# tnibler/local-features

Hardware: AMD Instinct MI355X
Metric: MKD descriptors/sec (32x32 patch, 128-D) (higher is better)
Workload: dtype f32 (f16x3 split MFMA pooling)

## Files before the change

local-features_amd/csrc/mkd_ablate.h:

```cpp
#pragma once
#include <hip/hip_runtime.h>

namespace lfmkd {
namespace ablate {

#ifdef LF_ABLATE_BLOAD
constexpr bool kNoFragmentReads = true;
#else
constexpr bool kNoFragmentReads = false;
#endif
#ifdef LF_ABLATE_SPLIT
constexpr bool kNoSplit = true;
#else
constexpr bool kNoSplit = false;
#endif
#ifdef LF_ABLATE_MMA
constexpr bool kNoMma = true;
#else
constexpr bool kNoMma = false;
#endif
#ifdef LF_ABLATE_FRONT
constexpr bool kNoFrontEnd = true;
#else
constexpr bool kNoFrontEnd = false;
#endif
#ifdef LF_ABLATE_MUL_FIRST_TAP
constexpr bool kMulFirstTap = true;
#else
constexpr bool kMulFirstTap = false;
#endif
#ifdef LF_ABLATE_SYNC
constexpr bool kNoRowSync = true;
#else
constexpr bool kNoRowSync = false;
#endif
#ifdef LF_ABLATE_EPILOGUE
constexpr bool kNoEpilogue = true;
#else
constexpr bool kNoEpilogue = false;
#endif
#ifdef LF_ABLATE_FORCE_W4
constexpr bool kForceFourWaves = true;
#else
constexpr bool kForceFourWaves = false;
#endif
#ifdef LF_KP_ABLATE_PRODUCER
constexpr bool kNoProducer = true;
#else
constexpr bool kNoProducer = false;
#endif
#ifdef LF_KP_ABLATE_TAPS
constexpr bool kNoTaps = true;
#else
constexpr bool kNoTaps = false;
#endif
#ifdef LF_KP_PRODUCER_PRIO
constexpr int kProducerPrio = LF_KP_PRODUCER_PRIO;
#else
constexpr int kProducerPrio = 2;
#endif
#ifdef LF_KP_CONSUMER_PRIO
constexpr int kConsumerPrio = LF_KP_CONSUMER_PRIO;
#else
constexpr int kConsumerPrio = -1;
#endif

#ifdef LF_ABLATE_ROWS
constexpr int kRows = LF_ABLATE_ROWS;
#else
constexpr int kRows = 32;
#endif

#ifdef LF_PHASE_TIMING
constexpr bool kPhaseTiming = true;
#else
constexpr bool kPhaseTiming = false;
#endif
struct PhaseClock {
    unsigned long long clk[8] = {0, 0, 0, 0, 0, 0, 0, 0}, prev = 0;
    __device__ __forceinline__ void start() {
        if constexpr (kPhaseTiming) prev = __builtin_readcyclecounter();
    }
    __device__ __forceinline__ void mark(int i) {
        if constexpr (kPhaseTiming) {
            __builtin_amdgcn_sched_barrier(0);
            const unsigned long long t = __builtin_readcyclecounter();
            clk[i] += t - prev;
            prev = t;
            __builtin_amdgcn_sched_barrier(0);
        }
    }
    __device__ __forceinline__ void dump(float *out, int wave, int lane) const {
        if constexpr (kPhaseTiming) {
            __syncthreads();
            if (blockIdx.x == 0 && lane == 0)
                for (int i = 0; i < 8; ++i) out[wave * 128 + i] = (float)clk[i];
        }
    }
};

}
}
```

local-features_amd/csrc/mkd_describe.hip:

```cpp
#include <hip/hip_runtime.h>
#include <stdint.h>

#include <type_traits>

#include "mkd_ablate.h"
#include "mkd_device.h"
#include "mkd_sample.h"

namespace lfmkd {


namespace {

typedef _Float16 f16x8 __attribute__((ext_vector_type(8)));
typedef unsigned int u32x4 __attribute__((ext_vector_type(4)));
typedef float f32x2 __attribute__((ext_vector_type(2)));
__device__ __forceinline__ f32x2 pk_fma(f32x2 a, f32x2 b, f32x2 c) { return __builtin_elementwise_fma(a, b, c); }
__device__ __forceinline__ f32x2 pk_set(float v) { return f32x2{v, v}; }

__device__ __host__ constexpr bool f16_family(int pool) { return pool == LF_POOL_F16X3 || pool == LF_POOL_F16_FP6; }

__device__ __host__ constexpr bool fold_form(int pool) { return pool != LF_POOL_F16_FP6; }
constexpr int kTiles = 21;
constexpr int kAccTiles = 21, kUnfAccTiles = 24;
__device__ __host__ constexpr int acc_tiles(bool fold) { return fold ? kAccTiles : kUnfAccTiles; }
__device__ __host__ constexpr int lut_pieces(bool fold) { return fold ? 24 : 30; }
__device__ __host__ constexpr bool valu_odd_cart(int pool) { return pool == LF_POOL_F16X3; }
constexpr int kOddCartSums = 7;
constexpr int kPolarSlots = 10;

constexpr float kB0 = 0.0096f, kB1 = 0.2054f, kB2 = 0.5699f;

__device__ __host__ constexpr int row_bytes(bool fold) { return lut_pieces(fold) * 1024; }
__device__ __host__ constexpr int ring_off(bool fold) { return 2 * row_bytes(fold); }
constexpr int kRowBytes = row_bytes(true), kRingOff = ring_off(true);
constexpr int kRingSlots = 6;
[[maybe_unused]] constexpr int kSrcPatches = 0, kSrcKeypoints = 1, kSrcKeypointsSplit = 2;
constexpr int kRingSlotsKp = 12;
constexpr int kLevelTableBytes = 5 * kMaxPyrLevels * 4;

__device__ __forceinline__ float lane_fetch(int byte_addr, float v) {
    return __int_as_float(__builtin_amdgcn_ds_bpermute(byte_addr, __float_as_int(v)));
}

__device__ __forceinline__ void lds_dma16(const void *gsrc, void *ldst) {
    __builtin_amdgcn_global_load_lds((const __attribute__((address_space(1))) void *)gsrc,
                                     (__attribute__((address_space(3))) void *)ldst, 16, 0, 0);
}
__device__ __forceinline__ void lds_dma16_sv(const unsigned char *uniform_base, unsigned lane_off, void *ldst) {
    asm("" : "+s"(uniform_base));
    asm volatile("" : "+v"(lane_off));
    lds_dma16(uniform_base + lane_off, ldst);
}

template <int W, bool FOLD, bool ODDV>
__device__ __forceinline__ void issue_lut_row(const unsigned char *__restrict__ lut_rows, int row,
                                              unsigned char *lds_row, int wave, int lane) {
    static_assert(!ODDV || FOLD, "the folded forms' tiles");
    constexpr int kPieces = ODDV ? lut_pieces(FOLD) - 8 : lut_pieces(FOLD);
    const unsigned lane16 = (unsigned)lane * 16u;
#pragma unroll
    for (int j = 0; j < (kPieces + W - 1) / W; ++j) {
        if (kPieces % W == 0 || wave + W * j < kPieces) {
            const int i = wave + W * j, piece = ODDV ? i + 2 * (i >> 2) : i;
            const unsigned char *g = lut_rows + ((size_t)row * row_bytes(FOLD) + (size_t)piece * 1024);
            lds_dma16_sv(g, lane16, lds_row + piece * 1024);
        }
    }
}

constexpr int kWStepBytes = 16384;
__device__ __forceinline__ constexpr int wstage_slot(int step) { return step % 3 == 0 ? 0 : (step % 3 == 1 ? 32768 : 16384); }
static_assert(wstage_slot(0) + kWStepBytes <= row_bytes(true) && wstage_slot(10) >= row_bytes(false) &&
              wstage_slot(10) + kWStepBytes <= 2 * row_bytes(true), "both forms' row buffers");

template <int W>
__device__ __forceinline__ void issue_w_step(const unsigned char *__restrict__ wfrag, int step, unsigned char *lds,
                                             int wave, int lane) {
    const unsigned lane16 = (unsigned)lane * 16u;
    unsigned char *d = lds + wstage_slot(step);
#pragma unroll
    for (int j = 0; j < 16 / W; ++j) {
        const unsigned char *g = wfrag + ((size_t)step * kWStepBytes + (size_t)(wave + W * j) * 1024);
        lds_dma16_sv(g, lane16, d + (wave + W * j) * 1024);
    }
}

template <int N> __device__ __forceinline__ void wait_vmcnt() { asm volatile("s_waitcnt vmcnt(%0)" ::"n"(N) : "memory"); }

struct RawSrc { const unsigned char *base; unsigned lane_off; };
__device__ __forceinline__ constexpr int clamp_row(int row) { return row < 0 ? 0 : (row > 31 ? 31 : row); }
__device__ __forceinline__ void issue_raw_row(const RawSrc &src, int row, unsigned char *ring, int slot) {
    const unsigned char *g = src.base + row * 128;
    lds_dma16_sv(g, src.lane_off, ring + slot * 2048);
    lds_dma16_sv(g + 64, src.lane_off, ring + slot * 2048 + 1024);
}

#pragma clang fp contract(off)

__device__ __forceinline__ float max3_tiny(float a, float b) {
    return __builtin_fmaxf(__builtin_fmaxf(a, b), 1e-30f);
}

template <int ANGLE>
__device__ __forceinline__ void gradient_direction(f32x2 gx, f32x2 gy, f32x2 r2, f32x2 &ct, f32x2 &st) {
    if (ANGLE == LF_ANGLE_EXACT || ANGLE == LF_ANGLE_EXACT_ZERO) {
        const f32x2 inv = {__builtin_amdgcn_rsqf(r2.x), __builtin_amdgcn_rsqf(r2.y)};
        const f32x2 c = gx * inv, s = -gy * inv;
        const bool z0 = ANGLE == LF_ANGLE_EXACT ? r2.x == 0.f : gx.x == 0.f;
        const bool z1 = ANGLE == LF_ANGLE_EXACT ? r2.y == 0.f : gx.y == 0.f;
        ct = f32x2{z0 ? 1.f : c.x, z1 ? 1.f : c.y};
        st = f32x2{z0 ? 0.f : s.x, z1 ? 0.f : s.y};
    } else {
        const float ax0 = fabsf(gx.x), ay0 = fabsf(gy.x), ax1 = fabsf(gx.y), ay1 = fabsf(gy.y);
        const bool sw0 = ax0 < ay0 && gx.x != 0.f, sw1 = ax1 < ay1 && gx.y != 0.f;
        const f32x2 mn = {__builtin_fminf(ax0, ay0), __builtin_fminf(ax1, ay1)};
        const f32x2 mx = {max3_tiny(ax0, ay0), max3_tiny(ax1, ay1)};
        const f32x2 a = mn * f32x2{__builtin_amdgcn_rcpf(mx.x), __builtin_amdgcn_rcpf(mx.y)};
        const f32x2 s = a * a;
        f32x2 p = pk_fma(s, pk_set(-0.0117212f), pk_set(0.05265332f));
        p = pk_fma(s, p, pk_set(-0.11643287f));
        p = pk_fma(s, p, pk_set(0.19354346f));
        p = pk_fma(s, p, pk_set(-0.33262347f));
        p = pk_fma(s, p, pk_set(0.99997726f));
        p = a * p;
        const f32x2 p2 = p * p;
        f32x2 sn = pk_fma(p2, pk_set(-0.000195038549f), pk_set(0.0083320355f));
        sn = pk_fma(p2, sn, pk_set(-0.166666508f));
        sn = pk_fma(p2, sn, pk_set(1.f));
        sn = p * sn;
        f32x2 cs = pk_fma(p2, pk_set(-0.00135857589f), pk_set(0.0416550152f));
        cs = pk_fma(p2, cs, pk_set(-0.499998569f));
        cs = pk_fma(p2, cs, pk_set(1.f));
        const unsigned sgn = 0x80000000u;
        float cr0 = __uint_as_float(__float_as_uint(sw0 ? sn.x : cs.x) | (__float_as_uint(gx.x) & sgn));
        float cr1 = __uint_as_float(__float_as_uint(sw1 ? sn.y : cs.y) | (__float_as_uint(gx.y) & sgn));
        float sr0 = __uint_as_float(__float_as_uint(sw0 ? cs.x : sn.x) | (~__float_as_uint(gy.x) & sgn));
        float sr1 = __uint_as_float(__float_as_uint(sw1 ? cs.y : sn.y) | (~__float_as_uint(gy.y) & sgn));
        ct = f32x2{cr0, cr1};
        st = f32x2{sr0, sr1};
    }
}

template <int ANGLE>
__device__ __forceinline__ void gradient_direction4(const f32x2 (&gx)[4], const f32x2 (&gy)[4], const f32x2 (&r2)[4],
                                                    f32x2 (&ct)[4], f32x2 (&st)[4]) {
    if (ANGLE != LF_ANGLE_SHADER) {
#pragma unroll
        for (int e = 0; e < 4; ++e) gradient_direction<ANGLE>(gx[e], gy[e], r2[e], ct[e], st[e]);
        return;
    }
    f32x2 a[4], s[4], p[4], p2[4], sn[4], cs[4];
    bool sw0[4], sw1[4];
#pragma unroll
    for (int e = 0; e < 4; ++e) {
        const float ax0 = fabsf(gx[e].x), ay0 = fabsf(gy[e].x), ax1 = fabsf(gx[e].y), ay1 = fabsf(gy[e].y);
        sw0[e] = ax0 < ay0 && gx[e].x != 0.f;
        sw1[e] = ax1 < ay1 && gx[e].y != 0.f;
        const f32x2 mn = {__builtin_fminf(ax0, ay0), __builtin_fminf(ax1, ay1)};
        const f32x2 mx = {max3_tiny(ax0, ay0), max3_tiny(ax1, ay1)};
        a[e] = mn * f32x2{__builtin_amdgcn_rcpf(mx.x), __builtin_amdgcn_rcpf(mx.y)};
    }
#pragma unroll
    for (int e = 0; e < 4; ++e) s[e] = a[e] * a[e];
#pragma unroll
    for (int e = 0; e < 4; ++e) p[e] = pk_fma(s[e], pk_set(-0.0117212f), pk_set(0.05265332f));
#pragma unroll
    for (int e = 0; e < 4; ++e) p[e] = pk_fma(s[e], p[e], pk_set(-0.11643287f));
#pragma unroll
    for (int e = 0; e < 4; ++e) p[e] = pk_fma(s[e], p[e], pk_set(0.19354346f));
#pragma unroll
    for (int e = 0; e < 4; ++e) p[e] = pk_fma(s[e], p[e], pk_set(-0.33262347f));
#pragma unroll
    for (int e = 0; e < 4; ++e) p[e] = pk_fma(s[e], p[e], pk_set(0.99997726f));
#pragma unroll
    for (int e = 0; e < 4; ++e) p[e] = a[e] * p[e];
#pragma unroll
    for (int e = 0; e < 4; ++e) p2[e] = p[e] * p[e];
// ... 200 lines not shown
    float ext[12];
    const float l0 = lane_fetch(addr_l, vb[6]), l1 = lane_fetch(addr_l, vb[7]);
    const float r0 = lane_fetch(addr_r, vb[0]), r1 = lane_fetch(addr_r, vb[1]);
    ext[0] = has_l ? l0 : vb[0];
    ext[1] = has_l ? l1 : vb[0];
    ext[10] = has_r ? r0 : vb[7];
    ext[11] = has_r ? r1 : vb[7];
#pragma unroll
    for (int x = 0; x < 8; ++x) ext[2 + x] = vb[x];
#pragma unroll
    for (int x = 0; x < 8; ++x) {
        float s = ablate::kMulFirstTap ? kB0 * ext[x] : fmaf(kB0, ext[x], 0.0f);
        s = fmaf(kB1, ext[x + 1], s);
        s = fmaf(kB2, ext[x + 2], s);
        s = fmaf(kB1, ext[x + 3], s);
        s = fmaf(kB0, ext[x + 4], s);
        out[x] = s;
    }
    const float hl = lane_fetch(addr_l, out[7]), hr = lane_fetch(addr_r, out[0]);
    out_l = has_l ? hl : out[0];
    out_r = has_r ? hr : out[7];
}

template <class SlotOfTap>
__device__ __forceinline__ void blur_row_impl(const unsigned char *ring_lane, SlotOfTap slot_of_tap, int addr_l, int addr_r,
                                              bool has_l, bool has_r, float (&out)[8], float &out_l, float &out_r) {
    float vb[8];
    vblur_row(ring_lane, ring_lane + 256, slot_of_tap, vb);
    hblur_row(vb, addr_l, addr_r, has_l, has_r, out, out_l, out_r);
}

__device__ __forceinline__ void hblur_row_fold(const float (&v)[8], int addr_l, int addr_r, bool has_l, bool has_r,
                                               float (&out)[8], float (&nb)[4]) {
    if constexpr (ablate::kNoFrontEnd) {
#pragma unroll
        for (int x = 0; x < 4; ++x) { out[x] = v[x]; out[4 + x] = v[7 - x]; }
        nb[0] = out[0]; nb[1] = out[3]; nb[2] = out[7]; nb[3] = out[4];
        return;
    }
    const float va[4] = {v[0], v[1], v[2], v[3]}, vb[4] = {v[4], v[5], v[6], v[7]};
    float ea[8], eb[8];
    {
        const float la0 = lane_fetch(addr_l, va[2]), la1 = lane_fetch(addr_l, va[3]);
        const float rb0 = lane_fetch(addr_l, vb[0]), rb1 = lane_fetch(addr_l, vb[1]);
        const float ra0 = lane_fetch(addr_r, va[0]), ra1 = lane_fetch(addr_r, va[1]);
        const float lb0 = lane_fetch(addr_r, vb[2]), lb1 = lane_fetch(addr_r, vb[3]);
        ea[0] = has_l ? la0 : va[0];
        ea[1] = has_l ? la1 : va[0];
        ea[6] = has_r ? ra0 : vb[0];
        ea[7] = has_r ? ra1 : vb[1];
        eb[0] = has_r ? lb0 : va[2];
        eb[1] = has_r ? lb1 : va[3];
        eb[6] = has_l ? rb0 : vb[3];
        eb[7] = has_l ? rb1 : vb[3];
    }
#pragma unroll
    for (int x = 0; x < 4; ++x) { ea[2 + x] = va[x]; eb[2 + x] = vb[x]; }
    float ob[4];
#pragma unroll
    for (int x = 0; x < 4; ++x) {
        float s = ablate::kMulFirstTap ? kB0 * ea[x] : fmaf(kB0, ea[x], 0.0f);
        s = fmaf(kB1, ea[x + 1], s);
        s = fmaf(kB2, ea[x + 2], s);
        s = fmaf(kB1, ea[x + 3], s);
        s = fmaf(kB0, ea[x + 4], s);
        out[x] = s;
        float t = ablate::kMulFirstTap ? kB0 * eb[x] : fmaf(kB0, eb[x], 0.0f);
        t = fmaf(kB1, eb[x + 1], t);
        t = fmaf(kB2, eb[x + 2], t);
        t = fmaf(kB1, eb[x + 3], t);
        t = fmaf(kB0, eb[x + 4], t);
        ob[x] = t;
    }
#pragma unroll
    for (int x = 0; x < 4; ++x) out[4 + x] = ob[3 - x];
    const float hal = lane_fetch(addr_l, out[3]), hbr = lane_fetch(addr_l, ob[0]);
    const float har = lane_fetch(addr_r, out[0]), hbl = lane_fetch(addr_r, ob[3]);
    nb[0] = has_l ? hal : out[0];
    nb[1] = has_r ? har : ob[0];
    nb[2] = has_r ? hbl : out[3];
    nb[3] = has_l ? hbr : ob[3];
}

template <class SlotOfTap>
__device__ __forceinline__ void blur_row_fold_impl(const unsigned char *ring_a, const unsigned char *ring_b, SlotOfTap slot_of_tap,
                                                   int addr_l, int addr_r, bool has_l, bool has_r, float (&out)[8],
                                                   float (&nb)[4]) {
    float v[8];
    vblur_row(ring_a, ring_b, slot_of_tap, v);
    hblur_row_fold(v, addr_l, addr_r, has_l, has_r, out, nb);
}

__device__ __forceinline__ void fold_sum(const f32x2 (&s)[4], f32x2 &e0, f32x2 &e1) { e0 = s[0] + s[2]; e1 = s[1] + s[3]; }
__device__ __forceinline__ void fold_diff(const f32x2 (&s)[4], f32x2 &o0, f32x2 &o1) { o0 = s[0] - s[2]; o1 = s[1] - s[3]; }
__device__ __forceinline__ void fold_diff_rev(const f32x2 (&s)[4], f32x2 &o0, f32x2 &o1) { o0 = s[2] - s[0]; o1 = s[3] - s[1]; }

__device__ __forceinline__ void odd_cart_row(const f32x2 (&fx)[2], const f32x4 &gy, f32x2 h0, f32x2 h1, float (&oc)[3]) {
    const f32x2 r = pk_fma(fx[1], h1, fx[0] * h0);
    const float t = r.x + r.y;
#pragma unroll
    for (int b = 0; b < 3; ++b) oc[b] = __builtin_fmaf(gy[b], t, oc[b]);
}

__device__ __forceinline__ void rebuild_odd_cart(const float (&oc)[kOddCartSums][3], int lane, f32x4 (&acc)[kAccTiles]) {
    constexpr float kVm[4] = {0.37872374f, 0.51796234f, 0.46882015f, 0.39798096f};
    asm volatile("" : "+v"(lane));
#pragma unroll
    for (int s = 0; s < kOddCartSums; ++s) {
        const int k = (s + 1) / 2, t = s == 0 ? 2 : 3 + 6 * (k - 1) + 4 + ((s - 1) & 1);
        f32x4 d = {0.f, 0.f, 0.f, 0.f};
#pragma unroll
        for (int b = 0; b < 3; ++b)
            d = __builtin_amdgcn_mfma_f32_16x16x4f32((lane & 15) == b ? kVm[k] : 0.f, oc[s][b], d, 0, 0, 0);
        acc[t] = d;
    }
}

template <int POOL>
__device__ __forceinline__ void pool_harmonics(const f32x2 (&m)[4], const f32x2 (&c1)[4], const f32x2 (&s1)[4],
                                               const unsigned char *brow, BFrag &g, f32x4 (&acc)[kAccTiles],
                                               const f32x2 (&fx)[2], const f32x4 &gy, float (&oc)[kOddCartSums][3]) {
    f32x2 pk[4], qk[4], pp[4], qp[4], tc[4];
    AFrag<POOL> au, av;
#pragma unroll
    for (int e = 0; e < 4; ++e) { pk[e] = m[e] * c1[e]; qk[e] = m[e] * s1[e]; tc[e] = c1[e] + c1[e]; }
#pragma unroll
    for (int k = 0; k < 3; ++k) {
        {
            f32x2 u[4], v[4];
            fold_sum(pk, u[0], u[1]);
            fold_diff(qk, u[2], u[3]);
            fold_sum(qk, v[0], v[1]);
            fold_diff_rev(pk, v[2], v[3]);
            if constexpr (valu_odd_cart(POOL)) {
                odd_cart_row(fx, gy, u[2], u[3], oc[1 + 2 * k]);
                odd_cart_row(fx, gy, v[2], v[3], oc[2 + 2 * k]);
            }
            if constexpr (POOL == LF_POOL_F16X3) {
                AFrag<POOL>::set2(au, u, av, v);
            } else {
                au.set(u);
                av.set(v);
            }
        }
        if (k < 2) {
#pragma unroll
            for (int e = 0; e < 4; ++e) {
                const f32x2 pn = pk_fma(tc[e], pk[e], k == 0 ? -m[e] : -pp[e]);
                const f32x2 qn = k == 0 ? tc[e] * qk[e] : pk_fma(tc[e], qk[e], -qp[e]);
                pp[e] = pk[e]; qp[e] = qk[e];
                pk[e] = pn; qk[e] = qn;
            }
        }
        const int a0 = 3 + 6 * k, u0 = 3 + 3 * k;
        const BFrag t0 = g, t1 = load_b(brow, u0 + 1);
        if constexpr (valu_odd_cart(POOL)) {
            if (k < 2) g = load_b(brow, u0 + 3);
            mma_part<POOL, 0>(au, t0, acc[a0 + 0]); mma_part<POOL, 0>(av, t0, acc[a0 + 1]); mma_part<POOL, 0>(au, t1, acc[a0 + 2]);
            mma_part<POOL, 0>(av, t1, acc[a0 + 3]);
            mma_part<POOL, 1>(au, t0, acc[a0 + 0]); mma_part<POOL, 1>(av, t0, acc[a0 + 1]); mma_part<POOL, 1>(au, t1, acc[a0 + 2]);
            mma_part<POOL, 1>(av, t1, acc[a0 + 3]);
            mma_part<POOL, 2>(au, t0, acc[a0 + 0]); mma_part<POOL, 2>(av, t0, acc[a0 + 1]); mma_part<POOL, 2>(au, t1, acc[a0 + 2]);
            mma_part<POOL, 2>(av, t1, acc[a0 + 3]);
            continue;
        }
        const BFrag t2 = load_b(brow, u0 + 2);
// ... 473 lines not shown
};
__device__ __forceinline__ RowSpan row_span(int role, int n_roles) {
    RowSpan sp;
    sp.lo = 32 * role / n_roles;
    sp.hi = 32 * (role + 1) / n_roles;
    const int r_first = sp.lo - 3 > 0 ? sp.lo - 3 : 0, r_last = sp.hi + 2 < 31 ? sp.hi + 2 : 31;
    sp.q_first = 4 * (r_first >> 2);
    sp.q_end = 4 * ((r_last >> 2) + 1);
    sp.n_pro = sp.lo == 0 ? 7 : 11;
    sp.consumer = role == n_roles - 1;
    return sp;
}

template <int W>
__device__ __forceinline__ void kp_produce_split(const KpSource &ks, const LevelTable &lt, const long *lvl_offset, long n,
                                                 long batch, const RowSpan &sp, unsigned char *s_mem,
                                                 const unsigned char *__restrict__ lut_rows, int pw, int lane) {
    __builtin_amdgcn_s_setprio(ablate::kProducerPrio);
    KpSampler<W> sm(ks, lt, lvl_offset, n, s_mem, pw, lane);
    KpTaps ta, tb;
    sm.load_geometry(batch, 0);
    sm.request(sp.q_first, 0, ta);
#pragma unroll 1
    for (int i = 0; i + 1 < sp.n_pro; i += 2) {
        sm.request(sp.q_first + i + 1, 0, tb);
        sm.finish(sp.q_first + i, 0, 0, ta);
        sm.request(sp.q_first + i + 2, 0, ta);
        sm.finish(sp.q_first + i + 1, 0, 0, tb);
    }
    sm.finish(sp.q_first + sp.n_pro - 1, 0, 0, ta);
    const int q_step0 = sp.q_first + sp.n_pro;
    if (q_step0 < sp.q_end) sm.request(q_step0, 0, ta);
    auto step = [&](int st, KpTaps &cur, KpTaps &nxt) {
        asm volatile("s_waitcnt vmcnt(0) lgkmcnt(0)" ::: "memory");
        __syncthreads();
        if (sp.lo + st + 1 < sp.hi) issue_lut_row<W, true, true>(lut_rows, sp.lo + st + 1, s_mem + ((st + 1) & 1) * kRowBytes, pw, lane);
        if (q_step0 + st + 1 < sp.q_end) sm.request(q_step0 + st + 1, 0, nxt);
        __builtin_amdgcn_sched_barrier(0);
        if (q_step0 + st < sp.q_end) sm.finish(q_step0 + st, 0, 0, cur);
    };
#pragma unroll 1
    for (int st = 0; st < sp.hi - sp.lo; st += 2) {
        step(st, ta, tb);
        step(st + 1, tb, ta);
    }
    asm volatile("s_waitcnt vmcnt(0) lgkmcnt(0)" ::: "memory");
    if (sp.consumer) {
#pragma unroll 1
        for (int e = 0; e < 12; ++e) __syncthreads();
    }
}

constexpr int kSplitSpinMax = 1 << 21;

}

template <int ANGLE, int POOL, int W, int SRC>
__global__ __launch_bounds__(SRC != kSrcPatches ? 128 * W : 64 * W) void mkd_pool(
    const float *__restrict__ patches, long n_host, const unsigned long long *__restrict__ n_dev,
    const unsigned char *__restrict__ lut_rows, const short *__restrict__ colmap, const unsigned char *__restrict__ wfrag,
    const float *__restrict__ bias, const float *__restrict__ odd_cart, float *__restrict__ out, float *__restrict__ raw_out,
    std::conditional_t<SRC != kSrcPatches, KpSource, int> ks, unsigned long long *__restrict__ clk) {
    constexpr bool kKp = SRC != kSrcPatches, kSplit = SRC == kSrcKeypointsSplit;
    static_assert(!kSplit || W == 2, "the row-split form is the narrow (2 + 2 wave) form");
    if (clk && blockIdx.x == 0 && threadIdx.x == 0) {
        clk[0] = __builtin_readcyclecounter();
        clk[1] = __builtin_amdgcn_s_memrealtime();
    }
    constexpr int kSlots = kKp ? kRingSlotsKp : kRingSlots;
    static_assert(!kKp || POOL == LF_POOL_F16X3, "keypoint mode pools in f16x3");
    constexpr int kMPool = POOL == LF_POOL_F16_FP6 ? LF_POOL_F16X3 : POOL;
    constexpr bool kFold = fold_form(POOL), kOddV = valu_odd_cart(POOL);
    constexpr bool kPairs = SRC == kSrcPatches && POOL == LF_POOL_F16X3;
    static_assert(!kKp || (kFold && kOddV), "the producers write the folded forms' LDS map and request f16x3's LUT pieces");
    constexpr int kNAcc = acc_tiles(kFold), kRowB = row_bytes(kFold), kRingO = ring_off(kFold);
    __shared__ __attribute__((aligned(16))) unsigned char s_mem[kRingO + W * kSlots * 2048 +
                                                                (kKp ? kLevelTableBytes + kMaxPyrLevels * 8 : 0)];
    const long n = n_dev ? (long)*n_dev : n_host;
    const int lane = threadIdx.x & 63;
    const int wave = __builtin_amdgcn_readfirstlane(threadIdx.x >> 6);
    const int p = lane & 15, q = lane >> 4;
    const int addr_l = ((lane - 16) & 63) * 4, addr_r = ((lane + 16) & 63) * 4;
    const bool has_l = q > 0, has_r = q < 3;
    const long nbatch = (n + 16 * W - 1) / (16 * W);
    unsigned char *ring = s_mem + kRingO + wave * (kSlots * 2048);
    BatchWalk walk{(long)blockIdx.x, nbatch, (long)gridDim.x};
    [[maybe_unused]] RowSpan span{0, 32, 0, 32, 7, true};
    [[maybe_unused]] int role = 0, n_roles = 1;
    if constexpr (kKp) {
        if constexpr (kSplit) {
            n_roles = ks.split;
            const long id = blockIdx.x, grp = id / (8 * n_roles), in = id - grp * (8 * n_roles);
            role = (int)(in >> 3);
            const long b = grp * 8 + (in & 7);
            walk = BatchWalk{b, b < nbatch ? b + 1 : b, 1};
            span = row_span(role, n_roles);
        } else {
            walk = kp_batches(nbatch);
        }
        if (walk.cur >= walk.end) return;
        int *lv = reinterpret_cast<int *>(s_mem + kRingO + W * kSlots * 2048);
        long *lv_off = reinterpret_cast<long *>(lv + 5 * kMaxPyrLevels);
        if (threadIdx.x < kMaxPyrLevels) {
            const int l = threadIdx.x;
            int w_ = 0, h_ = 0, pi_ = 0, ap_ = 0;
            long of_ = 0;
#pragma unroll
            for (int j = 0; j < kMaxPyrLevels; ++j)
                if (j == l) { w_ = ks.pd.w[j]; h_ = ks.pd.h[j]; pi_ = ks.pd.pitch[j]; ap_ = ks.pd.apron[j]; of_ = ks.pd.offset[j]; }
            lv[l] = w_; lv[kMaxPyrLevels + l] = h_; lv[2 * kMaxPyrLevels + l] = pi_; lv[3 * kMaxPyrLevels + l] = ap_;
            lv_off[l] = of_;
        }
        __syncthreads();
        const LevelTable lt{ks.pd.levels, lv, lv + kMaxPyrLevels, lv + 2 * kMaxPyrLevels, lv + 3 * kMaxPyrLevels};
        if (wave >= W) {
            if constexpr (kSplit) kp_produce_split<W>(ks, lt, lv_off, n, walk.cur, span, s_mem, lut_rows, wave - W, lane);
            else kp_produce<W>(ks, lt, lv_off, n, walk, s_mem, lut_rows, wave - W, lane);
            return;
        }

        if constexpr (ablate::kConsumerPrio >= 0) __builtin_amdgcn_s_setprio(ablate::kConsumerPrio);
    }
    const unsigned char *ring_lane = kFold ? ring + (q * 16 + p) * 16 : ring + (q >> 1) * 1024 + ((2 * (q & 1)) * 16 + p) * 16;
    [[maybe_unused]] const unsigned char *ring_mirror = ring + 1024 + ((3 - q) * 16 + p) * 16;

    long batch = walk.cur;
    if (batch >= walk.end) return;
    [[maybe_unused]] f32x2 oc_fx[2] = {pk_set(0.f), pk_set(0.f)};
    if constexpr (kOddV) {
        const f32x4 f = *reinterpret_cast<const f32x4 *>(odd_cart + 4 * q);
        oc_fx[0] = f32x2{f[0], f[1]};
        oc_fx[1] = f32x2{f[2], f[3]};
        asm volatile("" : "+v"(oc_fx[0]), "+v"(oc_fx[1]));
    }
    auto raw_src = [&](const float *pt, long b) {
        const long b0 = b * (16 * W) + wave * 16;
        const long wave0 = b0 < n ? b0 : n - 1;
        const long pidx = b0 + p < n ? b0 + p : n - 1;
        return RawSrc{reinterpret_cast<const unsigned char *>(pt + wave0 * 1024), (unsigned)(pidx - wave0) * 4096u + 16u * q};
    };
    {
        if constexpr (!kKp) {
            const RawSrc src = raw_src(patches, batch);
            if constexpr (kPairs) {
#pragma unroll
                for (int r = 0; r < kRingSlots; ++r) issue_raw_row(src, r, ring, r);
            } else {
#pragma unroll
                for (int r = -2; r <= 3; ++r) issue_raw_row(src, clamp_row(r), ring, r + 2);
            }
        }
        issue_lut_row<W, kFold, kOddV>(lut_rows, kSplit ? span.lo : 0, s_mem, wave, lane);
    }
    int slot0 = 0;
    unsigned par = 0;
    ablate::PhaseClock phase;
    phase.start();

    for (; batch < walk.end; batch += walk.step) {
        const unsigned char *wf = wfrag, *lr = lut_rows;
        const float *bs = bias, *pt = patches;
        float *o = out, *ro = raw_out;
        const short *cm = colmap;
        asm volatile("" : "+s"(wf), "+s"(bs), "+s"(lr), "+s"(o), "+s"(ro), "+s"(cm), "+s"(pt));
        const float *oc_tab = odd_cart;
        const long base = batch * (16 * W) + wave * 16;
        const bool more = batch + walk.step < walk.end;
        const RawSrc src = kKp ? RawSrc{nullptr, 0u} : raw_src(pt, batch);
        const RawSrc src_next = !kKp && more ? raw_src(pt, batch + walk.step) : src;

        f32x4 acc[kNAcc];
#pragma unroll
        for (int t = 0; t < kNAcc; ++t) acc[t] = f32x4{0.f, 0.f, 0.f, 0.f};
        [[maybe_unused]] float oc[kOddCartSums][3];
#pragma unroll
        for (int s = 0; s < kOddCartSums; ++s)
#pragma unroll
            for (int b = 0; b < 3; ++b) oc[s][b] = 0.f;
        float cur[8], prv[8], cur_nb[4] = {0.f, 0.f, 0.f, 0.f};
        [[maybe_unused]] float vnext[8];
        [[maybe_unused]] bool last_six = false;
        [[maybe_unused]] int s0 = 1;

        auto patch_row = [&](auto kind, const int g, auto pos) __attribute__((always_inline)) {
            constexpr bool kFirst = decltype(kind)::value == 0, kLast = decltype(kind)::value == 2;
            constexpr bool kFirstInner = decltype(kind)::value == 3;
            constexpr int kPos = decltype(pos)::value;
            constexpr bool kPairFirst = kPos >= 0 && (kPos & 1) == 0, kPairSecond = kPos >= 0 && (kPos & 1) == 1;
            constexpr int kSlot0 = kPos >= 0 ? (kPos & ~1) : 0;
            static_assert(kPairs ? (kFirst || kLast) == (kPos < 0) : kPos < 0, "the pair forms' rows 1..30 go in pairs");

            phase.mark(7);
            if constexpr (!ablate::kNoRowSync) {
                asm volatile("s_waitcnt vmcnt(0)" ::: "memory");
                __syncthreads();
            }
            phase.mark(0);
            const unsigned char *brow = s_mem + par * kRowB + lane * 16;
            if (f16_family(POOL) ? !kLast : (!kLast || more)) {
                if constexpr (!kKp) issue_lut_row<W, kFold, kOddV>(lr, (g + 1) & 31, s_mem + (par ^ 1) * kRowB, wave, lane);
            } else if (f16_family(POOL)) {
                issue_w_step<W>(wf, 0, s_mem, wave, lane);
            }
            par ^= 1;
            constexpr int kMTiles = kOddV ? 2 : 3;
            BFrag bm[kMTiles];
#pragma unroll
            for (int t = 0; t < kMTiles; ++t) bm[t] = load_b(brow, t);
            [[maybe_unused]] f32x4 oc_gy = {0.f, 0.f, 0.f, 0.f};
            if constexpr (kOddV) oc_gy = *reinterpret_cast<const f32x4 *>(oc_tab + 16 + 4 * g);

            if constexpr (!kKp && !kPairs)
                if (!kFirst && !kLast && g <= 29) issue_raw_row(src, clamp_row(g + 4), ring, s0 == 0 ? kRingSlots - 1 : s0 - 1);
            float nxt[8], nxt_nb[4] = {0.f, 0.f, 0.f, 0.f};
            if constexpr (!kPairs) {
                auto kp_slot = [&](int y, int i) {
                    int r_ = y - 2 + i;
                    r_ = r_ < 0 ? 0 : (r_ > 31 ? 31 : r_);
                    return (slot0 + r_) % kRingSlotsKp;
                };
                auto blur = [&](auto tap, float (&o)[8], float (&o_nb)[4]) __attribute__((always_inline)) {
                    if constexpr (kFold) blur_row_fold_impl(ring_lane, ring_mirror, tap, addr_l, addr_r, has_l, has_r, o, o_nb);
                    else blur_row_impl(ring_lane, tap, addr_l, addr_r, has_l, has_r, o, o_nb[0], o_nb[1]);
                };
                auto ring_tap = [](int first) {
                    return [first](int i) { const int sl = first + i; return sl >= kRingSlots ? sl - kRingSlots : sl; };
                };
                if (kFirst) {
                    if constexpr (kKp) blur([&](int i) { return kp_slot(0, i); }, cur, cur_nb);
                    else blur(ring_tap(0), cur, cur_nb);
#pragma unroll
                    for (int x = 0; x < 8; ++x) prv[x] = cur[x];
                }
                if constexpr (kFirstInner) {
                    float edge[4];
                    blur([&](int i) { return kp_slot(g - 1, i); }, prv, edge);
                    blur([&](int i) { return kp_slot(g, i); }, cur, cur_nb);
                }
                if (!kLast) {
                    if constexpr (kKp) blur([&](int i) { return kp_slot(g + 1, i); }, nxt, nxt_nb);
                    else blur(ring_tap(s0), nxt, nxt_nb);
                }
            } else {
                const unsigned char *ring_b = kFold ? ring_mirror : ring_lane + 256;
                auto hblur = [&](const float (&v)[8], float (&o)[8], float (&o_nb)[4]) __attribute__((always_inline)) {
                    if constexpr (kFold) hblur_row_fold(v, addr_l, addr_r, has_l, has_r, o, o_nb);
                    else hblur_row(v, addr_l, addr_r, has_l, has_r, o, o_nb[0], o_nb[1]);
                };
                auto slot = [](int j) { return (kSlot0 + j) % kRingSlots; };
                if constexpr (kFirst) {
                    float v0[8];
                    vblur_pair<4>(ring_lane, ring_b, slot, [](int i) { return i < 2 ? 0 : i - 2; },
                                  [](int i) { return i < 1 ? 0 : i - 1; }, v0, vnext);
                    hblur(v0, cur, cur_nb);
#pragma unroll
                    for (int x = 0; x < 8; ++x) prv[x] = cur[x];
                    hblur(vnext, nxt, nxt_nb);
                } else if constexpr (kPairFirst) {
                    float v1[8];
                    if (kPos == 4 && last_six)
                        vblur_pair<4>(ring_lane, ring_b, slot, [](int i) { return i < 3 ? i : 3; },
                                      [](int i) { return i < 2 ? i + 1 : 3; }, v1, vnext);
                    else
                        vblur_pair<6>(ring_lane, ring_b, slot, [](int i) { return i; }, [](int i) { return i + 1; }, v1, vnext);
                    asm volatile("s_waitcnt lgkmcnt(0)" ::: "memory");
                    if (!last_six || kPos == 0) {
                        issue_raw_row(src, g + 5, ring, kSlot0);
                        issue_raw_row(src, g + 6, ring, kSlot0 + 1);
                    } else if (more) {
                        if constexpr (kPos == 2) {
                            issue_raw_row(src_next, 2, ring, 2);
                            issue_raw_row(src_next, 3, ring, 3);
                        } else {
#pragma unroll
                            for (int r = 0; r < kRingSlots; ++r)
                                if (r != 2 && r != 3) issue_raw_row(src_next, r, ring, r);
                        }
                    }
                    hblur(v1, nxt, nxt_nb);
                } else if constexpr (kPairSecond) {
                    hblur(vnext, nxt, nxt_nb);
                }
            }
            if (kLast) {
#pragma unroll
                for (int x = 0; x < 8; ++x) nxt[x] = cur[x];
#pragma unroll
                for (int x = 0; x < 4; ++x) nxt_nb[x] = cur_nb[x];
            }
            asm volatile("" ::: "memory");
            if constexpr (!kKp && !kPairs) {
                if (kFirst) {
                    issue_raw_row(src, g + 4, ring, s0 == 0 ? kRingSlots - 1 : s0 - 1);
                } else if (kLast && more) {
#pragma unroll
                    for (int r = -2; r <= 3; ++r) issue_raw_row(src_next, clamp_row(r), ring, r + 2);
                }
                s0 = s0 == kRingSlots - 1 ? 0 : s0 + 1;
            }
            phase.mark(1);

            f32x2 m[4], c1[4], s1[4];
            {
                f32x2 gx[4], gy[4], r2n[4];
#pragma unroll
                for (int e = 0; e < 4; ++e) {
                    const int x = 2 * e;
                    f32x2 left, right;
                    if constexpr (kFold) {
                        left = e == 0 ? f32x2{cur_nb[0], cur[0]} : e == 1 ? f32x2{cur[1], cur[2]}
                               : e == 2 ? f32x2{cur[5], cur[6]} : f32x2{cur[7], cur_nb[2]};
                        right = e == 0 ? f32x2{cur[1], cur[2]} : e == 1 ? f32x2{cur[3], cur_nb[1]}
                                : e == 2 ? f32x2{cur_nb[3], cur[4]} : f32x2{cur[5], cur[6]};
                    } else {
                        left = f32x2{x == 0 ? cur_nb[0] : cur[x - 1], cur[x]};
                        right = f32x2{cur[x + 1], x == 6 ? cur_nb[1] : cur[x + 2]};
                    }
                    gx[e] = (left - right) + pk_set(0.0f);
                    gy[e] = f32x2{nxt[x], nxt[x + 1]} - f32x2{prv[x], prv[x + 1]};
                    r2n[e] = pk_fma(gy[e], gy[e], gx[e] * gx[e]);
                    const f32x2 r2 = r2n[e] + pk_set(1e-8f);
                    m[e] = f32x2{__builtin_amdgcn_sqrtf(__builtin_amdgcn_sqrtf(r2.x)),
                                 __builtin_amdgcn_sqrtf(__builtin_amdgcn_sqrtf(r2.y))};
                }
                if constexpr (ablate::kNoFrontEnd) {
#pragma unroll
                    for (int e = 0; e < 4; ++e) { c1[e] = gx[e]; s1[e] = gy[e]; }
                } else {
                    gradient_direction4<ANGLE>(gx, gy, r2n, c1, s1);
                }
            }
#pragma unroll
            for (int x = 0; x < 8; ++x) {
                prv[x] = cur[x];
                cur[x] = nxt[x];
            }
#pragma unroll
            for (int x = 0; x < 4; ++x) cur_nb[x] = nxt_nb[x];
            phase.mark(2);

            BFrag gfrag = load_b(brow, 3);
            {
                AFrag<kMPool> am;
                if constexpr (kFold) {
                    f32x2 mf[4];
                    fold_sum(m, mf[0], mf[1]);
                    fold_diff(m, mf[2], mf[3]);
                    if constexpr (kOddV) odd_cart_row(oc_fx, oc_gy, mf[2], mf[3], oc[0]);
                    am.set(mf);
                } else {
                    am.set(m);
                }
#pragma unroll
                for (int t = 0; t < kMTiles; ++t) mma_part<kMPool, 0>(am, bm[t], acc[t]);
#pragma unroll
                for (int t = 0; t < kMTiles; ++t) mma_part<kMPool, 1>(am, bm[t], acc[t]);
#pragma unroll
                for (int t = 0; t < kMTiles; ++t) mma_part<kMPool, 2>(am, bm[t], acc[t]);
            }
            phase.mark(3);
            if constexpr (POOL == LF_POOL_F16_FP6) pool_harmonics_fp6(m, c1, s1, brow, gfrag, acc);
            else pool_harmonics<POOL>(m, c1, s1, brow, gfrag, acc, oc_fx, oc_gy, oc);
            phase.mark(4);
            if constexpr (kPairs)
#pragma unroll
                for (int s = 0; s < kOddCartSums; ++s) asm volatile("" : "+v"(oc[s][0]), "+v"(oc[s][1]), "+v"(oc[s][2]));
            phase.mark(5);
        };
        constexpr std::integral_constant<int, -1> kOwnBody{};
        if constexpr (kSplit) {
            if (span.lo == 0) patch_row(std::integral_constant<int, 0>(), 0, kOwnBody);
            else patch_row(std::integral_constant<int, 3>(), span.lo, kOwnBody);
#pragma unroll 1
            for (int g = span.lo + 1; g < span.hi - 1; ++g) patch_row(std::integral_constant<int, 1>(), g, kOwnBody);
            if (span.consumer) patch_row(std::integral_constant<int, 2>(), span.hi - 1, kOwnBody);
            else patch_row(std::integral_constant<int, 1>(), span.hi - 1, kOwnBody);
            if constexpr (kOddV) rebuild_odd_cart(oc, lane, acc);
            unsigned *cnt = ks.xchg_cnt + batch * W + wave;
            typedef unsigned long long u64;
            if (!span.consumer) {
                u64 *dst = reinterpret_cast<u64 *>(ks.xchg + ((((long)batch * (n_roles - 1) + role) * W + wave) * kAccTiles) * 256) + lane;
#pragma unroll
                for (int t = 0; t < kAccTiles; ++t) {
                    const u64 v0 = ((u64)__float_as_uint(acc[t][1]) << 32) | __float_as_uint(acc[t][0]);
                    const u64 v1 = ((u64)__float_as_uint(acc[t][3]) << 32) | __float_as_uint(acc[t][2]);
                    __hip_atomic_store(dst + t * 128, v0, __ATOMIC_RELAXED, __HIP_MEMORY_SCOPE_AGENT);
                    __hip_atomic_store(dst + t * 128 + 64, v1, __ATOMIC_RELAXED, __HIP_MEMORY_SCOPE_AGENT);
                }
                asm volatile("s_waitcnt vmcnt(0)" ::: "memory");
                if (lane == 0) __hip_atomic_fetch_add(cnt, 1u, __ATOMIC_RELAXED, __HIP_MEMORY_SCOPE_AGENT);
                if (clk && blockIdx.x == 0 && threadIdx.x == 0) {
                    clk[2] = __builtin_readcyclecounter();
                    clk[3] = __builtin_amdgcn_s_memrealtime();
                }
                return;
            }
            int polls = 0;
            while (__hip_atomic_load(cnt, __ATOMIC_RELAXED, __HIP_MEMORY_SCOPE_AGENT) != (unsigned)(n_roles - 1) &&
                   polls < kSplitSpinMax) {
                __builtin_amdgcn_s_sleep(1);
                ++polls;
// ... 167 lines not shown
```

Measured before the change: 302.6 million.

## Exchange horizontal-blur halos through per-lane LDS records instead of bpermute

```diff
diff --git a/local-features_amd/csrc/mkd_ablate.h b/local-features_amd/csrc/mkd_ablate.h
--- a/local-features_amd/csrc/mkd_ablate.h
+++ b/local-features_amd/csrc/mkd_ablate.h
@@ -43,6 +43,11 @@
 constexpr bool kForceFourWaves = true;
 #else
 constexpr bool kForceFourWaves = false;
+#endif
+#ifdef LF_ABLATE_ROW_DMA
+constexpr bool kNoRowDma = true;
+#else
+constexpr bool kNoRowDma = false;
 #endif
 #ifdef LF_KP_ABLATE_PRODUCER
 constexpr bool kNoProducer = true;
diff --git a/local-features_amd/csrc/mkd_describe.hip b/local-features_amd/csrc/mkd_describe.hip
--- a/local-features_amd/csrc/mkd_describe.hip
+++ b/local-features_amd/csrc/mkd_describe.hip
@@ -47,13 +47,15 @@
     __builtin_amdgcn_global_load_lds((const __attribute__((address_space(1))) void *)gsrc,
                                      (__attribute__((address_space(3))) void *)ldst, 16, 0, 0);
 }
+template <bool LIVE = true>
 __device__ __forceinline__ void lds_dma16_sv(const unsigned char *uniform_base, unsigned lane_off, void *ldst) {
     asm("" : "+s"(uniform_base));
     asm volatile("" : "+v"(lane_off));
-    lds_dma16(uniform_base + lane_off, ldst);
-}
-
-template <int W, bool FOLD, bool ODDV>
+    if constexpr (LIVE) lds_dma16(uniform_base + lane_off, ldst);
+    else asm volatile("" ::"s"(uniform_base), "v"(lane_off), "s"((unsigned)(size_t)(__attribute__((address_space(3))) void *)ldst) : "memory");
+}
+
+template <int W, bool FOLD, bool ODDV, bool LIVE = true>
 __device__ __forceinline__ void issue_lut_row(const unsigned char *__restrict__ lut_rows, int row,
                                               unsigned char *lds_row, int wave, int lane) {
     static_assert(!ODDV || FOLD, "the folded forms' tiles");
@@ -64,7 +66,7 @@
         if (kPieces % W == 0 || wave + W * j < kPieces) {
             const int i = wave + W * j, piece = ODDV ? i + 2 * (i >> 2) : i;
             const unsigned char *g = lut_rows + ((size_t)row * row_bytes(FOLD) + (size_t)piece * 1024);
-            lds_dma16_sv(g, lane16, lds_row + piece * 1024);
+            lds_dma16_sv<LIVE>(g, lane16, lds_row + piece * 1024);
         }
     }
 }
@@ -90,10 +92,11 @@
 
 struct RawSrc { const unsigned char *base; unsigned lane_off; };
 __device__ __forceinline__ constexpr int clamp_row(int row) { return row < 0 ? 0 : (row > 31 ? 31 : row); }
+template <bool LIVE = true>
 __device__ __forceinline__ void issue_raw_row(const RawSrc &src, int row, unsigned char *ring, int slot) {
     const unsigned char *g = src.base + row * 128;
-    lds_dma16_sv(g, src.lane_off, ring + slot * 2048);
-    lds_dma16_sv(g + 64, src.lane_off, ring + slot * 2048 + 1024);
+    lds_dma16_sv<LIVE>(g, src.lane_off, ring + slot * 2048);
+    lds_dma16_sv<LIVE>(g + 64, src.lane_off, ring + slot * 2048 + 1024);
 }
 
 #pragma clang fp contract(off)
@@ -460,6 +463,78 @@
     nb[3] = has_l ? hbr : ob[3];
 }
 
+constexpr int kRecBack = 256, kRecPlane = 1024;
+typedef __attribute__((address_space(3))) unsigned char lds_u8;
+typedef __attribute__((address_space(3))) f32x4 lds_f32x4;
+typedef __attribute__((address_space(3))) f32x2 lds_f32x2;
+struct Halo { f32x2 la, rb, ra, lb; };
+__device__ __forceinline__ Halo halo_records(const float (&v)[8], lds_u8 *rec) {
+    Halo h{pk_set(0.f), pk_set(0.f), pk_set(0.f), pk_set(0.f)};
+    if constexpr (ablate::kNoFrontEnd) return h;
+    lds_u8 *own = rec + kRecBack;
+    const lds_u8 *left = rec, *right = rec + 2 * kRecBack;
+    *reinterpret_cast<lds_f32x4 *>(own) = f32x4{v[0], v[1], v[2], v[3]};
+    *reinterpret_cast<lds_f32x4 *>(own + kRecPlane) = f32x4{v[4], v[5], v[6], v[7]};
+    asm volatile("" ::: "memory");
+    h.la = *reinterpret_cast<const lds_f32x2 *>(left + 8);
+    h.rb = *reinterpret_cast<const lds_f32x2 *>(left + kRecPlane);
+    h.ra = *reinterpret_cast<const lds_f32x2 *>(right);
+    h.lb = *reinterpret_cast<const lds_f32x2 *>(right + kRecPlane + 8);
+    asm volatile("" ::: "memory");
+    return h;
+}
+__device__ __forceinline__ void hblur_row_fold_rec(const float (&v)[8], const Halo &h, lds_u8 *rec, bool has_l, bool has_r,
+                                                   float (&out)[8], float (&nb)[4]) {
+    if constexpr (ablate::kNoFrontEnd) {
+#pragma unroll
+        for (int x = 0; x < 4; ++x) { out[x] = v[x]; out[4 + x] = v[7 - x]; }
+        nb[0] = out[0]; nb[1] = out[3]; nb[2] = out[7]; nb[3] = out[4];
+        return;
+    }
+    const float va[4] = {v[0], v[1], v[2], v[3]}, vb[4] = {v[4], v[5], v[6], v[7]};
+    lds_u8 *own = rec + kRecBack;
+    const lds_u8 *left = rec, *right = rec + 2 * kRecBack;
+    const f32x2 la = h.la, rb = h.rb, ra = h.ra, lb = h.lb;
+    float ea[8], eb[8];
+    ea[0] = has_l ? la.x : va[0];
+    ea[1] = has_l ? la.y : va[0];
+    ea[6] = has_r ? ra.x : vb[0];
+    ea[7] = has_r ? ra.y : vb[1];
+    eb[0] = has_r ? lb.x : va[2];
+    eb[1] = has_r ? lb.y : va[3];
+    eb[6] = has_l ? rb.x : vb[3];
+    eb[7] = has_l ? rb.y : vb[3];
+#pragma unroll
+    for (int x = 0; x < 4; ++x) { ea[2 + x] = va[x]; eb[2 + x] = vb[x]; }
+    float ob[4];
+#pragma unroll
+    for (int x = 0; x < 4; ++x) {
+        float s = ablate::kMulFirstTap ? kB0 * ea[x] : fmaf(kB0, ea[x], 0.0f);
+        s = fmaf(kB1, ea[x + 1], s);
+        s = fmaf(kB2, ea[x + 2], s);
+        s = fmaf(kB1, ea[x + 3], s);
+        s = fmaf(kB0, ea[x + 4], s);
+        out[x] = s;
+        float t = ablate::kMulFirstTap ? kB0 * eb[x] : fmaf(kB0, eb[x], 0.0f);
+        t = fmaf(kB1, eb[x + 1], t);
+        t = fmaf(kB2, eb[x + 2], t);
+        t = fmaf(kB1, eb[x + 3], t);
+        t = fmaf(kB0, eb[x + 4], t);
+        ob[x] = t;
+    }
+#pragma unroll
+    for (int x = 0; x < 4; ++x) out[4 + x] = ob[3 - x];
+    *reinterpret_cast<lds_f32x4 *>(own) = f32x4{out[3], ob[0], out[0], ob[3]};
+    asm volatile("" ::: "memory");
+    const f32x2 el = *reinterpret_cast<const lds_f32x2 *>(left);
+    const f32x2 er = *reinterpret_cast<const lds_f32x2 *>(right + 8);
+    asm volatile("" ::: "memory");
+    nb[0] = has_l ? el.x : out[0];
+    nb[1] = has_r ? er.x : ob[0];
+    nb[2] = has_r ? er.y : out[3];
+    nb[3] = has_l ? el.y : ob[3];
+}
+
 template <class SlotOfTap>
 __device__ __forceinline__ void blur_row_fold_impl(const unsigned char *ring_a, const unsigned char *ring_b, SlotOfTap slot_of_tap,
                                                    int addr_l, int addr_r, bool has_l, bool has_r, float (&out)[8],
@@ -1099,6 +1174,8 @@
     const int p = lane & 15, q = lane >> 4;
     const int addr_l = ((lane - 16) & 63) * 4, addr_r = ((lane + 16) & 63) * 4;
     const bool has_l = q > 0, has_r = q < 3;
+    [[maybe_unused]] lds_u8 *rec = (lds_u8 *)s_mem + ((wave >> 2) * kRowB + (6 * (wave & 3) + 4) * 1024 + lane * 16 - kRecBack);
+    if constexpr (kPairs) asm volatile("" : "+v"(rec));
     const long nbatch = (n + 16 * W - 1) / (16 * W);
     unsigned char *ring = s_mem + kRingO + wave * (kSlots * 2048);
     BatchWalk walk{(long)blockIdx.x, nbatch, (long)gridDim.x};
@@ -1196,6 +1273,7 @@
             for (int b = 0; b < 3; ++b) oc[s][b] = 0.f;
         float cur[8], prv[8], cur_nb[4] = {0.f, 0.f, 0.f, 0.f};
         [[maybe_unused]] float vnext[8];
+        [[maybe_unused]] Halo hnext;
         [[maybe_unused]] bool last_six = false;
         [[maybe_unused]] int s0 = 1;
 
@@ -1206,6 +1284,7 @@
             constexpr bool kPairFirst = kPos >= 0 && (kPos & 1) == 0, kPairSecond = kPos >= 0 && (kPos & 1) == 1;
             constexpr int kSlot0 = kPos >= 0 ? (kPos & ~1) : 0;
             static_assert(kPairs ? (kFirst || kLast) == (kPos < 0) : kPos < 0, "the pair forms' rows 1..30 go in pairs");
+            constexpr bool kRowDma = !ablate::kNoRowDma;
 
             phase.mark(7);
             if constexpr (!ablate::kNoRowSync) {
@@ -1215,7 +1294,7 @@
             phase.mark(0);
             const unsigned char *brow = s_mem + par * kRowB + lane * 16;
             if (f16_family(POOL) ? !kLast : (!kLast || more)) {
-                if constexpr (!kKp) issue_lut_row<W, kFold, kOddV>(lr, (g + 1) & 31, s_mem + (par ^ 1) * kRowB, wave, lane);
+                if constexpr (!kKp) issue_lut_row<W, kFold, kOddV, kRowDma>(lr, (g + 1) & 31, s_mem + (par ^ 1) * kRowB, wave, lane);
             } else if (f16_family(POOL)) {
                 issue_w_step<W>(wf, 0, s_mem, wave, lane);
             }
@@ -1228,7 +1307,7 @@
             if constexpr (kOddV) oc_gy = *reinterpret_cast<const f32x4 *>(oc_tab + 16 + 4 * g);
 
             if constexpr (!kKp && !kPairs)
-                if (!kFirst && !kLast && g <= 29) issue_raw_row(src, clamp_row(g + 4), ring, s0 == 0 ? kRingSlots - 1 : s0 - 1);
+                if (!kFirst && !kLast && g <= 29) issue_raw_row<kRowDma>(src, clamp_row(g + 4), ring, s0 == 0 ? kRingSlots - 1 : s0 - 1);
             float nxt[8], nxt_nb[4] = {0.f, 0.f, 0.f, 0.f};
             if constexpr (!kPairs) {
                 auto kp_slot = [&](int y, int i) {
@@ -1261,7 +1340,7 @@
             } else {
                 const unsigned char *ring_b = kFold ? ring_mirror : ring_lane + 256;
                 auto hblur = [&](const float (&v)[8], float (&o)[8], float (&o_nb)[4]) __attribute__((always_inline)) {
-                    if constexpr (kFold) hblur_row_fold(v, addr_l, addr_r, has_l, has_r, o, o_nb);
+                    if constexpr (kFold) hblur_row_fold_rec(v, halo_records(v, rec), rec, has_l, has_r, o, o_nb);
                     else hblur_row(v, addr_l, addr_r, has_l, has_r, o, o_nb[0], o_nb[1]);
                 };
                 auto slot = [](int j) { return (kSlot0 + j) % kRingSlots; };
@@ -1282,21 +1361,23 @@
                         vblur_pair<6>(ring_lane, ring_b, slot, [](int i) { return i; }, [](int i) { return i + 1; }, v1, vnext);
                     asm volatile("s_waitcnt lgkmcnt(0)" ::: "memory");
                     if (!last_six || kPos == 0) {
-                        issue_raw_row(src, g + 5, ring, kSlot0);
-                        issue_raw_row(src, g + 6, ring, kSlot0 + 1);
+                        issue_raw_row<kRowDma>(src, g + 5, ring, kSlot0);
+                        issue_raw_row<kRowDma>(src, g + 6, ring, kSlot0 + 1);
                     } else if (more) {
                         if constexpr (kPos == 2) {
-                            issue_raw_row(src_next, 2, ring, 2);
-                            issue_raw_row(src_next, 3, ring, 3);
+                            issue_raw_row<kRowDma>(src_next, 2, ring, 2);
+                            issue_raw_row<kRowDma>(src_next, 3, ring, 3);
                         } else {
 #pragma unroll
                             for (int r = 0; r < kRingSlots; ++r)
-                                if (r != 2 && r != 3) issue_raw_row(src_next, r, ring, r);
+                                if (r != 2 && r != 3) issue_raw_row<kRowDma>(src_next, r, ring, r);
                         }
                     }
-                    hblur(v1, nxt, nxt_nb);
+                    const Halo h1 = halo_records(v1, rec);
+                    hnext = halo_records(vnext, rec);
+                    hblur_row_fold_rec(v1, h1, rec, has_l, has_r, nxt, nxt_nb);
                 } else if constexpr (kPairSecond) {
-                    hblur(vnext, nxt, nxt_nb);
+                    hblur_row_fold_rec(vnext, hnext, rec, has_l, has_r, nxt, nxt_nb);
                 }
             }
             if (kLast) {
@@ -1308,10 +1389,10 @@
             asm volatile("" ::: "memory");
             if constexpr (!kKp && !kPairs) {
                 if (kFirst) {
-                    issue_raw_row(src, g + 4, ring, s0 == 0 ? kRingSlots - 1 : s0 - 1);
+                    issue_raw_row<kRowDma>(src, g + 4, ring, s0 == 0 ? kRingSlots - 1 : s0 - 1);
                 } else if (kLast && more) {
 #pragma unroll
-                    for (int r = -2; r <= 3; ++r) issue_raw_row(src_next, clamp_row(r), ring, r + 2);
+                    for (int r = -2; r <= 3; ++r) issue_raw_row<kRowDma>(src_next, clamp_row(r), ring, r + 2);
                 }
                 s0 = s0 == kRingSlots - 1 ? 0 : s0 + 1;
             }
@@ -1333,7 +1414,8 @@
                         left = f32x2{x == 0 ? cur_nb[0] : cur[x - 1], cur[x]};
                         right = f32x2{cur[x + 1], x == 6 ? cur_nb[1] : cur[x + 2]};
                     }
-                    gx[e] = (left - right) + pk_set(0.0f);
+                    if constexpr (kPairs) gx[e] = f32x2{left.x - right.x, left.y - right.y} + pk_set(0.0f);
+                    else gx[e] = (left - right) + pk_set(0.0f);
                     gy[e] = f32x2{nxt[x], nxt[x + 1]} - f32x2{prv[x], prv[x + 1]};
                     r2n[e] = pk_fma(gy[e], gy[e], gx[e] * gx[e]);
                     const f32x2 r2 = r2n[e] + pk_set(1e-8f);
```

Measured after the change: 307.7 million (median of 6 runs). +1.7%, better.
